# zkonduit/ezkl

Hardware: NVIDIA H100
Metric: prove_time_s (lower is better)
Workload: dtype u32 limbs (254-bit Montgomery integers mod BN254 r/p)

## Files before the change

ezkl_b200/csrc/field.cuh:

```cuda
#pragma once
#include <stdint.h>
#include "fp_ptx.cuh"

#if defined(__CUDACC__)
#define HD __host__ __device__ __forceinline__
#define DEV __device__ __forceinline__
#else
#define HD inline
#define DEV inline
#endif

namespace b200 {

struct FrTag {
    static constexpr uint32_t INV = 0xefffffffu;
    HD static uint32_t mod(int i) {
        constexpr uint32_t M[8] = {0xf0000001u, 0x43e1f593u, 0x79b97091u, 0x2833e848u, 0x8181585du, 0xb85045b6u, 0xe131a029u, 0x30644e72u};
        return M[i];
    }
    HD static uint32_t one(int i) {
        constexpr uint32_t V[8] = {0x4ffffffbu, 0xac96341cu, 0x9f60cd29u, 0x36fc7695u, 0x7879462eu, 0x666ea36fu, 0x9a07df2fu, 0x0e0a77c1u};
        return V[i];
    }
    HD static uint32_t r2(int i) {
// ... 180 lines not shown
    {
        uint64_t br = 2;
        for (int i = 0; i < 8; ++i) { uint64_t s = (uint64_t)Tag::mod(i) - br; e[i] = (uint32_t)s; br = (s >> 32) & 1; }
    }
    Fp<Tag> acc = fp_one<Tag>();
#pragma unroll 1
    for (int i = 253; i >= 0; --i) {
        acc = acc * acc;
        if ((e[i >> 5] >> (i & 31)) & 1) acc = acc * a;
    }
    return acc;
}
template <class Tag> HD Fp<Tag> fp_pow_u64(const Fp<Tag>& a, uint64_t e) {
    Fp<Tag> acc = fp_one<Tag>();
#pragma unroll 1
    for (int i = 63; i >= 0; --i) {
        acc = acc * acc;
        if ((e >> i) & 1) acc = acc * a;
    }
    return acc;
}

#if defined(__CUDACC__)
template <class Tag> DEV Fp<Tag> fp_load(const Fp<Tag>* p) {
    Fp<Tag> r;
    const uint4* q = reinterpret_cast<const uint4*>(p);
    uint4 lo = q[0], hi = q[1];
    r.l[0] = lo.x; r.l[1] = lo.y; r.l[2] = lo.z; r.l[3] = lo.w;
    r.l[4] = hi.x; r.l[5] = hi.y; r.l[6] = hi.z; r.l[7] = hi.w;
    return r;
}
template <class Tag> DEV void fp_store(Fp<Tag>* p, const Fp<Tag>& v) {
    uint4* q = reinterpret_cast<uint4*>(p);
    q[0] = make_uint4(v.l[0], v.l[1], v.l[2], v.l[3]);
    q[1] = make_uint4(v.l[4], v.l[5], v.l[6], v.l[7]);
}
#endif

}
```

ezkl_b200/csrc/fp_gen.py:

```python
#!/usr/bin/env python
import random
import sys

M32 = 0xFFFFFFFF
FIELDS = {
    "fr": 0x30644e72e131a029b85045b68181585d2833e84879b9709143e1f593f0000001,
    "fq": 0x30644e72e131a029b85045b68181585d97816a916871ca8d3c208c16d87cfd47,
}


def limbs(x, n=8):
    return [(x >> (32 * i)) & M32 for i in range(n)]


def gen_mul(mod):
    Ml = limbs(mod)
    inv = (-pow(mod, -1, 1 << 32)) & M32
    ins = []
    X = ["x%d" % i for i in range(8)]
    Y = ["y%d" % i for i in range(8)]
    A = ["a%d" % i for i in range(8)]
    B = ["b%d" % i for i in range(8)]

    def imm(v):
        return "0x%08x" % v

    def reduce_row(E, O):
        ins.append(("mul.lo.u32", "m", E[0], imm(inv)))
        for j in range(4):
            ins.append((("mad.lo.cc.u32" if j == 0 else "madc.lo.cc.u32"), O[2 * j], "m", imm(Ml[2 * j + 1]), O[2 * j]))
            ins.append(("madc.hi.cc.u32", O[2 * j + 1], "m", imm(Ml[2 * j + 1]), O[2 * j + 1]))
        for j in range(4):
            ins.append((("mad.lo.cc.u32" if j == 0 else "madc.lo.cc.u32"), E[2 * j], "m", imm(Ml[2 * j]), E[2 * j]))
            ins.append(("madc.hi.cc.u32", E[2 * j + 1], "m", imm(Ml[2 * j]), E[2 * j + 1]))
        ins.append(("addc.u32", O[7], O[7], "0"))

    for j in range(4):
        ins.append(("mul.lo.u32", X[2 * j], A[2 * j], B[0]))
        ins.append(("mul.hi.u32", X[2 * j + 1], A[2 * j], B[0]))
    for j in range(4):
        ins.append(("mul.lo.u32", Y[2 * j], A[2 * j + 1], B[0]))
        ins.append(("mul.hi.u32", Y[2 * j + 1], A[2 * j + 1], B[0]))
    E, O = X, Y
    reduce_row(E, O)
    for i in range(1, 8):
        nE, nO = O, E
        ins.append(("add.cc.u32", nE[0], nE[0], nO[1]))
        for j in range(4):
            c_lo = nO[2 * j + 2] if 2 * j + 2 < 8 else "0"
            c_hi = nO[2 * j + 3] if 2 * j + 3 < 8 else "0"
            ins.append(("madc.lo.cc.u32", nO[2 * j], A[2 * j + 1], B[i], c_lo))
            ins.append(("madc.hi.cc.u32", nO[2 * j + 1], A[2 * j + 1], B[i], c_hi))
        for j in range(4):
            ins.append((("mad.lo.cc.u32" if j == 0 else "madc.lo.cc.u32"), nE[2 * j], A[2 * j], B[i], nE[2 * j]))
            ins.append(("madc.hi.cc.u32", nE[2 * j + 1], A[2 * j], B[i], nE[2 * j + 1]))
        ins.append(("addc.u32", nO[7], nO[7], "0"))
        E, O = nE, nO
        reduce_row(E, O)
    T = ["t%d" % i for i in range(8)]
    for j in range(7):
        ins.append((("add.cc.u32" if j == 0 else "addc.cc.u32"), T[j], O[j], E[j + 1]))
    ins.append(("addc.u32", T[7], O[7], "0"))
    ins += final_sub(T, Ml)
    return ins


def gen_mul2(mod):
    Ml = limbs(mod)
    inv = (-pow(mod, -1, 1 << 32)) & M32
    ins = []
    X = ["x%d" % i for i in range(8)]
    Y = ["y%d" % i for i in range(8)]
    A = ["a%d" % i for i in range(8)]
    B = ["b%d" % i for i in range(8)]
    Cc = ["c%d" % i for i in range(8)]
    D = ["d%d" % i for i in range(8)]

    def imm(v):
        return "0x%08x" % v

    def acc_rows(E, O, P, q):
        def pair(p):
            return (q, p) if p.startswith("0x") else (p, q)
        for j in range(4):
            ins.append((("mad.lo.cc.u32" if j == 0 else "madc.lo.cc.u32"), O[2 * j]) + pair(P[2 * j + 1]) + (O[2 * j],))
            ins.append(("madc.hi.cc.u32", O[2 * j + 1]) + pair(P[2 * j + 1]) + (O[2 * j + 1],))
# ... 109 lines not shown


def final_sub(T, Ml, out=None):
    out = out or ["r%d" % i for i in range(8)]
    ins = []
    S = ["s%d" % i for i in range(8)]
    for j in range(8):
        ins.append((("sub.cc.u32" if j == 0 else "subc.cc.u32"), S[j], T[j], "0x%08x" % Ml[j]))
    ins.append(("subc.u32", "brw", "0", "0"))
    ins.append(("setp.eq.u32", "p", "brw", "0"))
    for j in range(8):
        ins.append(("selp.u32", out[j], S[j], T[j], "p"))
    return ins


def gen_add(mod):
    Ml = limbs(mod)
    ins = []
    T = ["t%d" % i for i in range(8)]
    for j in range(8):
        op = "add.cc.u32" if j == 0 else ("addc.cc.u32" if j < 7 else "addc.u32")
        ins.append((op, T[j], "a%d" % j, "b%d" % j))
    return ins + final_sub(T, Ml)


def gen_sub(mod):
    Ml = limbs(mod)
    ins = []
    T = ["t%d" % i for i in range(8)]
    for j in range(8):
        ins.append((("sub.cc.u32" if j == 0 else "subc.cc.u32"), T[j], "a%d" % j, "b%d" % j))
    ins.append(("subc.u32", "brw", "0", "0"))
    for j in range(8):
        ins.append(("and.b32", "s%d" % j, "brw", "0x%08x" % Ml[j]))
    for j in range(8):
        op = "add.cc.u32" if j == 0 else ("addc.cc.u32" if j < 7 else "addc.u32")
        ins.append((op, "r%d" % j, T[j], "s%d" % j))
    return ins


def run(ins, regs):
    cc = 0
    pred = {}

    def val(x):
        if x in regs:
# ... 4 lines not shown
        op, d = it[0], it[1]
        s = [val(x) if x not in pred else x for x in it[2:]]
        if op == "mul.lo.u32":
            regs[d] = (s[0] * s[1]) & M32
        elif op == "mul.hi.u32":
            regs[d] = (s[0] * s[1]) >> 32
        elif op in ("mad.lo.cc.u32", "madc.lo.cc.u32", "madc.hi.cc.u32", "mad.hi.cc.u32"):
            p = s[0] * s[1]
            p = (p & M32) if ".lo" in op else (p >> 32)
            t = p + s[2] + (cc if op.startswith("madc") else 0)
            regs[d], cc = t & M32, t >> 32
        elif op in ("add.cc.u32", "addc.cc.u32", "addc.u32"):
            t = s[0] + s[1] + (cc if op.startswith("addc") else 0)
            regs[d] = t & M32
            if ".cc" in op:
                cc = t >> 32
        elif op in ("sub.cc.u32", "subc.cc.u32", "subc.u32"):
            t = s[0] - s[1] - (cc if op.startswith("subc") else 0)
            regs[d] = t & M32
            if ".cc" in op:
                cc = 1 if t < 0 else 0
        elif op == "and.b32":
            regs[d] = s[0] & s[1]
        elif op == "shl.b32":
            regs[d] = (s[0] << s[1]) & M32
        elif op == "shf.l.clamp.b32":
            regs[d] = ((((s[1] << 32) | s[0]) << min(s[2], 32)) >> 32) & M32
        elif op == "setp.eq.u32":
            pred[d] = (s[0] == s[1])
        elif op == "selp.u32":
            regs[d] = s[0] if pred[it[4]] else s[1]
        else:
            raise ValueError(op)
        assert 0 <= regs.get(d, 0) <= M32
    return regs


def check(name, mod, trials=3000):
    rng = random.Random(hash(name) & 0xFFFF)
    mul, add, sub = gen_mul(mod), gen_add(mod), gen_sub(mod)
    Rinv = pow(1 << 256, -1, mod)
    edge = [0, 1, 2, mod - 1, mod - 2, (1 << 254) % mod, (1 << 253), mod >> 1, 0xFFFFFFFF, (1 << 128) - 1]
    pairs = [(x, y) for x in edge for y in edge] + [(rng.randrange(mod), rng.randrange(mod)) for _ in range(trials)]
    for a, b in pairs:
        regs = {}
        for i, v in enumerate(limbs(a)):
# ... 7 lines not shown
    mul2 = gen_mul2(mod)
    edge2 = [0, 1, mod - 1, mod, (1 << 254) % mod, 0xFFFFFFFF, mod >> 1]
    quads = [(a, b, c, d) for a in edge2 for b in edge2 for c in edge2 for d in edge2]
    quads += [tuple(rng.randrange(mod) for _ in range(4)) for _ in range(trials)]
    for a, b, c, d in quads:
        regs = {}
        for nm, v in (("a", a), ("b", b), ("c", c), ("d", d)):
            for i, w in enumerate(limbs(v)):
                regs["%s%d" % (nm, i)] = w
        out = run(mul2, regs)
        got = sum(out["r%d" % i] << (32 * i) for i in range(8))
        exp = (a * b + c * d) * Rinv % mod
        assert got == exp, (name, "mul2", hex(a), hex(b), hex(c), hex(d), hex(got), hex(exp))
    sqr = gen_sqr(mod)
    for a in edge + [mod, (1 << 254) - 1 if (1 << 254) - 1 < mod else mod - 3, 0x80000000, 0xFFFFFFFF << 32, int("80000000" * 8, 16) % mod,
                     int("ffffffff" * 7, 16)] + [rng.randrange(mod) for _ in range(trials)]:
        regs = {"a%d" % i: v for i, v in enumerate(limbs(a))}
        out = run(sqr, regs)
        got = sum(out["r%d" % i] << (32 * i) for i in range(8))
        assert got == a * a * Rinv % mod, (name, "sqr", hex(a), hex(got))
    return len(mul), len(add), len(sub), len(mul2), len(sqr)


def emit_fn(fname, ins, n_in):
    tmp = sorted({x for it in ins for x in it[1:] if x[0] in "xytsmuw" and not x.startswith("0x")} | {"brw"})
    tmp = [t for t in tmp if t != "p"]
    lines = ["    .reg .u32 %s;" % ", ".join(tmp), "    .reg .pred p;"]

    def opnd(x):
        if x[0] == "r" and x[1:].isdigit():
            return "%%%d" % int(x[1:])
        if x[0] == "a" and x[1:].isdigit():
            return "%%%d" % (8 + int(x[1:]))
        if x[0] == "b" and x[1:].isdigit() and x != "brw":
            return "%%%d" % (16 + int(x[1:]))
        if x[0] == "c" and x[1:].isdigit():
            return "%%%d" % (24 + int(x[1:]))
        if x[0] == "d" and x[1:].isdigit():
            return "%%%d" % (32 + int(x[1:]))
        return x

    for it in ins:
        lines.append("    %s %s;" % (it[0], ", ".join(opnd(x) for x in it[1:])))
    body = "\n".join('        "%s\\n\\t"' % ln.strip() for ln in ["{"] + lines + ["}"])
    outs = ", ".join('"=r"(r[%d])' % i for i in range(8))
    inps = ", ".join('"r"(a[%d])' % i for i in range(8))
    args = "uint32_t* r, const uint32_t* a"
    if n_in >= 2:
        inps += ", " + ", ".join('"r"(b[%d])' % i for i in range(8))
        args += ", const uint32_t* b"
    if n_in == 4:
        inps += ", " + ", ".join('"r"(c[%d])' % i for i in range(8)) + ", " + ", ".join('"r"(d[%d])' % i for i in range(8))
        args += ", const uint32_t* c, const uint32_t* d"
    return ("__device__ __forceinline__ void %s(%s) {\n    asm(\n%s\n        : %s\n        : %s);\n}\n"
            % (fname, args, body, outs, inps))


def main():
    out = ["// GENERATED by fp_gen.py -- do not edit.  Every instruction list below was executed by the generator's",
           "// PTX interpreter against Python bigints (edge + random operands) before this file was written.",
           "#pragma once", "#include <stdint.h>", "#if defined(__CUDA_ARCH__)", ""]
    for name, mod in FIELDS.items():
        n = check(name, mod)
        print("%s: verified; instruction counts mul/add/sub/mul2/sqr = %s" % (name, n))
        out.append(emit_fn("%s_mul_ptx" % name, gen_mul(mod), 2))
        out.append(emit_fn("%s_add_ptx" % name, gen_add(mod), 2))
        out.append(emit_fn("%s_sub_ptx" % name, gen_sub(mod), 2))
        out.append(emit_fn("%s_mul2_ptx" % name, gen_mul2(mod), 4))
        out.append(emit_fn("%s_sqr_ptx" % name, gen_sqr(mod), 1))
    out.append("#endif  // __CUDA_ARCH__")
    if "--check" not in sys.argv:
        import os
        with open(os.path.join(os.path.dirname(os.path.abspath(__file__)), "fp_ptx.cuh"), "w") as f:
            f.write("\n".join(out) + "\n")


if __name__ == "__main__":
    main()
```

ezkl_b200/csrc/fp_ptx.cuh:

```cuda
#pragma once
#include <stdint.h>
#if defined(__CUDA_ARCH__)

__device__ __forceinline__ void fr_mul_ptx(uint32_t* r, const uint32_t* a, const uint32_t* b) {
    asm(
        "{\n\t"
        ".reg .u32 brw, m, s0, s1, s2, s3, s4, s5, s6, s7, t0, t1, t2, t3, t4, t5, t6, t7, x0, x1, x2, x3, x4, x5, x6, x7, y0, y1, y2, y3, y4, y5, y6, y7;\n\t"
        ".reg .pred p;\n\t"
        "mul.lo.u32 x0, %8, %16;\n\t"
        "mul.hi.u32 x1, %8, %16;\n\t"
        "mul.lo.u32 x2, %10, %16;\n\t"
        "mul.hi.u32 x3, %10, %16;\n\t"
        "mul.lo.u32 x4, %12, %16;\n\t"
        "mul.hi.u32 x5, %12, %16;\n\t"
        "mul.lo.u32 x6, %14, %16;\n\t"
        "mul.hi.u32 x7, %14, %16;\n\t"
        "mul.lo.u32 y0, %9, %16;\n\t"
        "mul.hi.u32 y1, %9, %16;\n\t"
        "mul.lo.u32 y2, %11, %16;\n\t"
        "mul.hi.u32 y3, %11, %16;\n\t"
        "mul.lo.u32 y4, %13, %16;\n\t"
        "mul.hi.u32 y5, %13, %16;\n\t"
        "mul.lo.u32 y6, %15, %16;\n\t"
        "mul.hi.u32 y7, %15, %16;\n\t"
// ... 2262 lines not shown
        "sub.cc.u32 s0, t0, 0xd87cfd47;\n\t"
        "subc.cc.u32 s1, t1, 0x3c208c16;\n\t"
        "subc.cc.u32 s2, t2, 0x6871ca8d;\n\t"
        "subc.cc.u32 s3, t3, 0x97816a91;\n\t"
        "subc.cc.u32 s4, t4, 0x8181585d;\n\t"
        "subc.cc.u32 s5, t5, 0xb85045b6;\n\t"
        "subc.cc.u32 s6, t6, 0xe131a029;\n\t"
        "subc.cc.u32 s7, t7, 0x30644e72;\n\t"
        "subc.u32 brw, 0, 0;\n\t"
        "setp.eq.u32 p, brw, 0;\n\t"
        "selp.u32 %0, s0, t0, p;\n\t"
        "selp.u32 %1, s1, t1, p;\n\t"
        "selp.u32 %2, s2, t2, p;\n\t"
        "selp.u32 %3, s3, t3, p;\n\t"
        "selp.u32 %4, s4, t4, p;\n\t"
        "selp.u32 %5, s5, t5, p;\n\t"
        "selp.u32 %6, s6, t6, p;\n\t"
        "selp.u32 %7, s7, t7, p;\n\t"
        "}\n\t"
        : "=r"(r[0]), "=r"(r[1]), "=r"(r[2]), "=r"(r[3]), "=r"(r[4]), "=r"(r[5]), "=r"(r[6]), "=r"(r[7])
        : "r"(a[0]), "r"(a[1]), "r"(a[2]), "r"(a[3]), "r"(a[4]), "r"(a[5]), "r"(a[6]), "r"(a[7]));
}

#endif
```

ezkl_b200/csrc/ntt.cu:

```cuda
#include <cstdlib>
#include "ntt.cuh"

namespace b200 {

struct PassArgs {
    const Fr* src; Fr* dst;
    size_t src_pstride, dst_pstride;
    uint32_t logm, log_g, inner_cnt, in_r_fast;
    uint64_t in_rs, in_inner_s, in_outer_s;
    uint64_t out_rs, out_inner_s, out_outer_s;
    uint64_t n_in;
    uint32_t tw_on, rest_is_inner, lo_bits, first, last;
    uint64_t tw_mul;
    const Fr* tw_m; const Fr* t_lo; const Fr* t_hi;
    const uint4* tw_staged;
    const Fr* t_full;
    NttScale pre, post;
    uint32_t pre_c0_is_one;
    uint32_t peer_on, log_slice, block0;
    const Fr* src_peers[8];
    Fr* dst_peers[8];
};

DEV Fr sh_get(const uint4* lo, const uint4* hi, uint32_t i) {
// ... 117 lines not shown
    }

    int s = (int)a.logm - 1;
    bool first = true, tw_ready = false;
    while (s >= 0) {
        const bool two = !(first && (a.logm & 1u));
        const int s_next = two ? s - 2 : s - 1;
        const bool last = s_next < 0;
        uint32_t g, t;
        const bool g_fast = last || (first && !a.in_r_fast);
        if (g_fast) { g = tid & (G - 1); t = tid >> a.log_g; } else { t = tid & (Q - 1); g = tid >> (a.logm - 2); }
        const uint32_t q = 1u << (s - 1), p = t & (q - 1), blk = t >> (s - 1);
        const uint32_t base = (blk << (s + 1)) + p;
        Fr x[4];
        const bool sparse = first && a.first && a.n_in < ((uint64_t)M * a.inner_cnt);
        if (first) {
#pragma unroll
            for (int j = 0; j < 4; ++j) {
                const uint64_t idx = in_base + (uint64_t)g * a.in_inner_s + (uint64_t)(base + j * q) * a.in_rs;
                x[j] = fp_zero<FrTag>();
                if (idx < a.n_in) {
                    x[j] = fp_load(a.peer_on ? a.src_peers[idx >> a.log_slice] + (idx & slice_mask) : src + idx);
                    if (a.first) {
                        if (a.pre.mode == 1) x[j] = x[j] * a.pre.c[0];
                        else if (a.pre.mode == 3) { uint32_t m3 = (uint32_t)(idx % 3); if (m3 || !a.pre_c0_is_one) x[j] = x[j] * a.pre.c[m3]; }
                    }
                }
            }
        } else {
#pragma unroll
            for (int j = 0; j < 4; ++j) x[j] = sh_get(dlo, dhi, (g << a.logm) + base + j * q);
        }
        if (!tw_ready) { mbar_wait(&bar, 0); tw_ready = true; }
        {
            const uint32_t o = (1u << s) - 1u;
            Fr u0 = x[0] + x[2], u2 = x[0] - x[2], u1 = x[1] + x[3], u3 = x[1] - x[3];
            if (s > 0) {
                if (p && !(sparse && fp_is_zero(u2))) u2 = u2 * sh_get(tlo, thi, o + p);
                if (!(sparse && fp_is_zero(u3))) u3 = u3 * sh_get(tlo, thi, o + p + q);
            }
            x[0] = u0; x[1] = u1; x[2] = u2; x[3] = u3;
        }
        if (two) {
            const uint32_t o = (1u << (s - 1)) - 1u;
            Fr v0 = x[0] + x[1], v1 = x[0] - x[1], v2 = x[2] + x[3], v3 = x[2] - x[3];
            if (s - 1 > 0 && p) {
                Fr w = sh_get(tlo, thi, o + p);
                if (!(sparse && fp_is_zero(v1))) v1 = v1 * w;
                if (!(sparse && fp_is_zero(v3))) v3 = v3 * w;
            }
            x[0] = v0; x[1] = v1; x[2] = v2; x[3] = v3;
        }
        if (!last) {
#pragma unroll
            for (int j = 0; j < 4; ++j) sh_put(dlo, dhi, (g << a.logm) + base + j * q, x[j]);
            __syncthreads();
        } else {
#pragma unroll
            for (int j = 0; j < 4; ++j) {
                const uint32_t pos = base + j * q;
                const uint32_t rp = __brev(pos) >> (32 - a.logm);
                Fr v = x[j];
                if (a.tw_on) {
                    const uint64_t i_rest = a.rest_is_inner ? (uint64_t)(inner0 + g) : 0;
                    const uint64_t ex = a.tw_mul * (uint64_t)rp * i_rest;
                    if (ex) {
                        if (a.t_full) v = v * fp_load(a.t_full + ex);
                        else {
                            const uint32_t elo = (uint32_t)(ex & ((1ull << a.lo_bits) - 1)), ehi = (uint32_t)(ex >> a.lo_bits);
                            Fr w = fp_load(a.t_lo + elo);
                            if (ehi) w = w * fp_load(a.t_hi + ehi);
                            v = v * w;
                        }
                    }
                }
                const uint64_t idx = out_base + (uint64_t)g * a.out_inner_s + (uint64_t)rp * a.out_rs;
                if (a.last) {
                    if (a.post.mode == 1) v = v * a.post.c[0];
                    else if (a.post.mode == 3) v = v * a.post.c[(uint32_t)(idx % 3)];
                }
                fp_store(a.peer_on ? a.dst_peers[idx >> a.log_slice] + (idx & slice_mask) : dst + idx, v);
            }
        }
        first = false;
        s = s_next;
    }
}

__global__ void k_stage_twiddles(Fr w, uint32_t logm, uint4* __restrict__ out) {
    const uint32_t M = 1u << logm, idx = blockIdx.x * blockDim.x + threadIdx.x;
    if (idx >= M) return;
    Fr v = fp_zero<FrTag>();
    if (idx + 1 < M) {
        const uint32_t s = 31 - __clz(idx + 1), p = idx + 1 - (1u << s);
        v = fp_pow_u64(w, (uint64_t)p << (logm - 1 - s));
    }
    out[idx] = make_uint4(v.l[0], v.l[1], v.l[2], v.l[3]);
    out[M + idx] = make_uint4(v.l[4], v.l[5], v.l[6], v.l[7]);
}
__global__ void k_powers_run(Fr base, uint64_t count, Fr* __restrict__ out) {
    const uint64_t i0 = ((uint64_t)blockIdx.x * blockDim.x + threadIdx.x) * 32;
    if (i0 >= count) return;
    Fr v = fp_pow_u64(base, i0);
    for (uint64_t i = i0; i < i0 + 32 && i < count; ++i) { fp_store(out + i, v); v = v * base; }
// ... 177 lines not shown
```

Before: 0.08531.

## Use lazy [0,2r) Montgomery reduction in NTT butterflies, canonicalize on store

Adds generated PTX for lazy Fr arithmetic: Montgomery multiply without the final conditional subtraction, add and sub that keep results in [0,2r), a reduce-mod-2r and a canonicalize step. The NTT kernel's butterflies, twiddle multiplies and pre/post scaling now use these lazy ops, with one canonicalization before each global store. The aim is to drop the per-op compare-and-select against r and shorten the instruction count per butterfly. The cost is extra reduce2 calls on the untwiddled branches and reliance on redundant-range correctness, which the generator checks by simulation.

```diff
diff --git a/ezkl_b200/csrc/field.cuh b/ezkl_b200/csrc/field.cuh
--- a/ezkl_b200/csrc/field.cuh
+++ b/ezkl_b200/csrc/field.cuh
@@ -226,6 +226,42 @@
 }
 
 #if defined(__CUDACC__)
+DEV Fr fr_mul_lazy(const Fr& a, const Fr& b) {
+    Fr r;
+#if defined(__CUDA_ARCH__)
+    fr_mul_lazy_ptx(r.l, a.l, b.l);
+#endif
+    return r;
+}
+DEV Fr fr_add_lazy(const Fr& a, const Fr& b) {
+    Fr r;
+#if defined(__CUDA_ARCH__)
+    fr_add_lazy_ptx(r.l, a.l, b.l);
+#endif
+    return r;
+}
+DEV Fr fr_sub_lazy(const Fr& a, const Fr& b) {
+    Fr r;
+#if defined(__CUDA_ARCH__)
+    fr_sub_lazy_ptx(r.l, a.l, b.l);
+#endif
+    return r;
+}
+DEV Fr fr_reduce2(const Fr& a) {
+    Fr r;
+#if defined(__CUDA_ARCH__)
+    fr_reduce2_ptx(r.l, a.l);
+#endif
+    return r;
+}
+DEV Fr fr_canonicalize(const Fr& a) {
+    Fr r;
+#if defined(__CUDA_ARCH__)
+    fr_canonicalize_ptx(r.l, a.l);
+#endif
+    return r;
+}
+
 template <class Tag> DEV Fp<Tag> fp_load(const Fp<Tag>* p) {
     Fp<Tag> r;
     const uint4* q = reinterpret_cast<const uint4*>(p);
diff --git a/ezkl_b200/csrc/fp_gen.py b/ezkl_b200/csrc/fp_gen.py
--- a/ezkl_b200/csrc/fp_gen.py
+++ b/ezkl_b200/csrc/fp_gen.py
@@ -13,7 +13,7 @@
     return [(x >> (32 * i)) & M32 for i in range(n)]
 
 
-def gen_mul(mod):
+def gen_mul(mod, lazy=False):
     Ml = limbs(mod)
     inv = (-pow(mod, -1, 1 << 32)) & M32
     ins = []
@@ -57,11 +57,12 @@
         ins.append(("addc.u32", nO[7], nO[7], "0"))
         E, O = nE, nO
         reduce_row(E, O)
-    T = ["t%d" % i for i in range(8)]
+    T = ["r%d" % i for i in range(8)] if lazy else ["t%d" % i for i in range(8)]
     for j in range(7):
         ins.append((("add.cc.u32" if j == 0 else "addc.cc.u32"), T[j], O[j], E[j + 1]))
     ins.append(("addc.u32", T[7], O[7], "0"))
-    ins += final_sub(T, Ml)
+    if not lazy:
+        ins += final_sub(T, Ml)
     return ins
 
 
@@ -217,6 +218,33 @@
         op = "add.cc.u32" if j == 0 else ("addc.cc.u32" if j < 7 else "addc.u32")
         ins.append((op, T[j], "a%d" % j, "b%d" % j))
     return ins + final_sub(T, Ml)
+
+
+def gen_add_lazy(mod):
+    ins = []
+    T = ["t%d" % i for i in range(8)]
+    for j in range(8):
+        op = "add.cc.u32" if j == 0 else ("addc.cc.u32" if j < 7 else "addc.u32")
+        ins.append((op, T[j], "a%d" % j, "b%d" % j))
+    return ins + final_sub(T, limbs(2 * mod))
+
+
+def gen_sub_lazy(mod):
+    M2 = limbs(2 * mod)
+    ins = []
+    T = ["t%d" % i for i in range(8)]
+    for j in range(8):
+        op = "sub.cc.u32" if j == 0 else ("subc.cc.u32" if j < 7 else "subc.u32")
+        ins.append((op, T[j], "a%d" % j, "b%d" % j))
+    for j in range(8):
+        op = "add.cc.u32" if j == 0 else ("addc.cc.u32" if j < 7 else "addc.u32")
+        ins.append((op, "r%d" % j, T[j], "0x%08x" % M2[j]))
+    return ins
+
+
+def gen_reduce(mod, k):
+    T = ["t%d" % i for i in range(8)]
+    return [("mov.b32", T[j], "a%d" % j) for j in range(8)] + final_sub(T, limbs(k * mod))
 
 
 def gen_sub(mod):
@@ -267,6 +295,8 @@
                 cc = 1 if t < 0 else 0
         elif op == "and.b32":
             regs[d] = s[0] & s[1]
+        elif op == "mov.b32":
+            regs[d] = s[0]
         elif op == "shl.b32":
             regs[d] = (s[0] << s[1]) & M32
         elif op == "shf.l.clamp.b32":
@@ -320,6 +350,41 @@
     return len(mul), len(add), len(sub), len(mul2), len(sqr)
 
 
+def check_lazy(name, mod, trials=3000):
+    rng = random.Random((hash(name) + 1) & 0xFFFF)
+    Rinv = pow(1 << 256, -1, mod)
+    mul, add, sub = gen_mul(mod, lazy=True), gen_add_lazy(mod), gen_sub_lazy(mod)
+    red2, canon = gen_reduce(mod, 2), gen_reduce(mod, 1)
+    edge = [0, mod - 1, mod, 2 * mod - 1]
+    edge4 = edge + [2 * mod, 3 * mod, 4 * mod - 1]
+
+    def go(ins, **ops):
+        regs = {}
+        for nm, v in ops.items():
+            for i, w in enumerate(limbs(v)):
+                regs["%s%d" % (nm, i)] = w
+        out = run(ins, regs)
+        return sum(out["r%d" % i] << (32 * i) for i in range(8))
+
+    two = [(a, b) for a in edge for b in edge] + [(rng.randrange(2 * mod), rng.randrange(2 * mod)) for _ in range(trials)]
+    for a, b in two:
+        got = go(mul, a=a, b=b)
+        assert got < 2 * mod and got % mod == a * b * Rinv % mod, (name, "mul_lazy", hex(a), hex(b), hex(got))
+        got = go(add, a=a, b=b)
+        assert got < 2 * mod and got % mod == (a + b) % mod, (name, "add_lazy", hex(a), hex(b), hex(got))
+        got = go(sub, a=a, b=b)
+        assert got == a - b + 2 * mod, (name, "sub_lazy", hex(a), hex(b), hex(got))
+    wide = [(a, b) for a in edge4 for b in (0, 1, mod - 1)] + [(rng.randrange(4 * mod), rng.randrange(mod)) for _ in range(trials)]
+    for a, b in wide:
+        got = go(mul, a=a, b=b)
+        assert got < 2 * mod and got % mod == a * b * Rinv % mod, (name, "mul_lazy 4M", hex(a), hex(b), hex(got))
+    for a in edge4 + [rng.randrange(4 * mod) for _ in range(trials)]:
+        assert go(red2, a=a) == a % (2 * mod), (name, "reduce 2M", hex(a))
+        if a < 2 * mod:
+            assert go(canon, a=a) == a % mod, (name, "canonicalize", hex(a))
+    return len(mul), len(add), len(sub), len(red2), len(canon)
+
+
 def emit_fn(fname, ins, n_in):
     tmp = sorted({x for it in ins for x in it[1:] if x[0] in "xytsmuw" and not x.startswith("0x")} | {"brw"})
     tmp = [t for t in tmp if t != "p"]
@@ -366,6 +431,13 @@
         out.append(emit_fn("%s_sub_ptx" % name, gen_sub(mod), 2))
         out.append(emit_fn("%s_mul2_ptx" % name, gen_mul2(mod), 4))
         out.append(emit_fn("%s_sqr_ptx" % name, gen_sqr(mod), 1))
+    n = check_lazy("fr", FIELDS["fr"])
+    print("fr lazy: verified; instruction counts mul/add/sub/reduce2/canonicalize = %s" % (n,))
+    out.append(emit_fn("fr_mul_lazy_ptx", gen_mul(FIELDS["fr"], lazy=True), 2))
+    out.append(emit_fn("fr_add_lazy_ptx", gen_add_lazy(FIELDS["fr"]), 2))
+    out.append(emit_fn("fr_sub_lazy_ptx", gen_sub_lazy(FIELDS["fr"]), 2))
+    out.append(emit_fn("fr_reduce2_ptx", gen_reduce(FIELDS["fr"], 2), 1))
+    out.append(emit_fn("fr_canonicalize_ptx", gen_reduce(FIELDS["fr"], 1), 1))
     out.append("#endif  // __CUDA_ARCH__")
     if "--check" not in sys.argv:
         import os
diff --git a/ezkl_b200/csrc/fp_ptx.cuh b/ezkl_b200/csrc/fp_ptx.cuh
--- a/ezkl_b200/csrc/fp_ptx.cuh
+++ b/ezkl_b200/csrc/fp_ptx.cuh
@@ -2308,4 +2308,442 @@
         : "r"(a[0]), "r"(a[1]), "r"(a[2]), "r"(a[3]), "r"(a[4]), "r"(a[5]), "r"(a[6]), "r"(a[7]));
 }
 
+__device__ __forceinline__ void fr_mul_lazy_ptx(uint32_t* r, const uint32_t* a, const uint32_t* b) {
+    asm(
+        "{\n\t"
+        ".reg .u32 brw, m, x0, x1, x2, x3, x4, x5, x6, x7, y0, y1, y2, y3, y4, y5, y6, y7;\n\t"
+        ".reg .pred p;\n\t"
+        "mul.lo.u32 x0, %8, %16;\n\t"
+        "mul.hi.u32 x1, %8, %16;\n\t"
+        "mul.lo.u32 x2, %10, %16;\n\t"
+        "mul.hi.u32 x3, %10, %16;\n\t"
+        "mul.lo.u32 x4, %12, %16;\n\t"
+        "mul.hi.u32 x5, %12, %16;\n\t"
+        "mul.lo.u32 x6, %14, %16;\n\t"
+        "mul.hi.u32 x7, %14, %16;\n\t"
+        "mul.lo.u32 y0, %9, %16;\n\t"
+        "mul.hi.u32 y1, %9, %16;\n\t"
+        "mul.lo.u32 y2, %11, %16;\n\t"
+        "mul.hi.u32 y3, %11, %16;\n\t"
+        "mul.lo.u32 y4, %13, %16;\n\t"
+        "mul.hi.u32 y5, %13, %16;\n\t"
+        "mul.lo.u32 y6, %15, %16;\n\t"
+        "mul.hi.u32 y7, %15, %16;\n\t"
+        "mul.lo.u32 m, x0, 0xefffffff;\n\t"
+        "mad.lo.cc.u32 y0, m, 0x43e1f593, y0;\n\t"
+        "madc.hi.cc.u32 y1, m, 0x43e1f593, y1;\n\t"
+        "madc.lo.cc.u32 y2, m, 0x2833e848, y2;\n\t"
+        "madc.hi.cc.u32 y3, m, 0x2833e848, y3;\n\t"
+        "madc.lo.cc.u32 y4, m, 0xb85045b6, y4;\n\t"
+        "madc.hi.cc.u32 y5, m, 0xb85045b6, y5;\n\t"
+        "madc.lo.cc.u32 y6, m, 0x30644e72, y6;\n\t"
+        "madc.hi.cc.u32 y7, m, 0x30644e72, y7;\n\t"
+        "mad.lo.cc.u32 x0, m, 0xf0000001, x0;\n\t"
+        "madc.hi.cc.u32 x1, m, 0xf0000001, x1;\n\t"
+        "madc.lo.cc.u32 x2, m, 0x79b97091, x2;\n\t"
+        "madc.hi.cc.u32 x3, m, 0x79b97091, x3;\n\t"
+        "madc.lo.cc.u32 x4, m, 0x8181585d, x4;\n\t"
+        "madc.hi.cc.u32 x5, m, 0x8181585d, x5;\n\t"
+        "madc.lo.cc.u32 x6, m, 0xe131a029, x6;\n\t"
+        "madc.hi.cc.u32 x7, m, 0xe131a029, x7;\n\t"
+        "addc.u32 y7, y7, 0;\n\t"
+        "add.cc.u32 y0, y0, x1;\n\t"
+        "madc.lo.cc.u32 x0, %9, %17, x2;\n\t"
+        "madc.hi.cc.u32 x1, %9, %17, x3;\n\t"
+        "madc.lo.cc.u32 x2, %11, %17, x4;\n\t"
+        "madc.hi.cc.u32 x3, %11, %17, x5;\n\t"
+        "madc.lo.cc.u32 x4, %13, %17, x6;\n\t"
+        "madc.hi.cc.u32 x5, %13, %17, x7;\n\t"
+        "madc.lo.cc.u32 x6, %15, %17, 0;\n\t"
+        "madc.hi.cc.u32 x7, %15, %17, 0;\n\t"
+        "mad.lo.cc.u32 y0, %8, %17, y0;\n\t"
+        "madc.hi.cc.u32 y1, %8, %17, y1;\n\t"
+        "madc.lo.cc.u32 y2, %10, %17, y2;\n\t"
+        "madc.hi.cc.u32 y3, %10, %17, y3;\n\t"
+        "madc.lo.cc.u32 y4, %12, %17, y4;\n\t"
+        "madc.hi.cc.u32 y5, %12, %17, y5;\n\t"
+        "madc.lo.cc.u32 y6, %14, %17, y6;\n\t"
+        "madc.hi.cc.u32 y7, %14, %17, y7;\n\t"
+        "addc.u32 x7, x7, 0;\n\t"
+        "mul.lo.u32 m, y0, 0xefffffff;\n\t"
+        "mad.lo.cc.u32 x0, m, 0x43e1f593, x0;\n\t"
+        "madc.hi.cc.u32 x1, m, 0x43e1f593, x1;\n\t"
+        "madc.lo.cc.u32 x2, m, 0x2833e848, x2;\n\t"
+        "madc.hi.cc.u32 x3, m, 0x2833e848, x3;\n\t"
+        "madc.lo.cc.u32 x4, m, 0xb85045b6, x4;\n\t"
+        "madc.hi.cc.u32 x5, m, 0xb85045b6, x5;\n\t"
+        "madc.lo.cc.u32 x6, m, 0x30644e72, x6;\n\t"
+        "madc.hi.cc.u32 x7, m, 0x30644e72, x7;\n\t"
+        "mad.lo.cc.u32 y0, m, 0xf0000001, y0;\n\t"
+        "madc.hi.cc.u32 y1, m, 0xf0000001, y1;\n\t"
+        "madc.lo.cc.u32 y2, m, 0x79b97091, y2;\n\t"
+        "madc.hi.cc.u32 y3, m, 0x79b97091, y3;\n\t"
+        "madc.lo.cc.u32 y4, m, 0x8181585d, y4;\n\t"
+        "madc.hi.cc.u32 y5, m, 0x8181585d, y5;\n\t"
+        "madc.lo.cc.u32 y6, m, 0xe131a029, y6;\n\t"
+        "madc.hi.cc.u32 y7, m, 0xe131a029, y7;\n\t"
+        "addc.u32 x7, x7, 0;\n\t"
+        "add.cc.u32 x0, x0, y1;\n\t"
+        "madc.lo.cc.u32 y0, %9, %18, y2;\n\t"
+        "madc.hi.cc.u32 y1, %9, %18, y3;\n\t"
+        "madc.lo.cc.u32 y2, %11, %18, y4;\n\t"
+        "madc.hi.cc.u32 y3, %11, %18, y5;\n\t"
+        "madc.lo.cc.u32 y4, %13, %18, y6;\n\t"
+        "madc.hi.cc.u32 y5, %13, %18, y7;\n\t"
+        "madc.lo.cc.u32 y6, %15, %18, 0;\n\t"
+        "madc.hi.cc.u32 y7, %15, %18, 0;\n\t"
+        "mad.lo.cc.u32 x0, %8, %18, x0;\n\t"
+        "madc.hi.cc.u32 x1, %8, %18, x1;\n\t"
+        "madc.lo.cc.u32 x2, %10, %18, x2;\n\t"
+        "madc.hi.cc.u32 x3, %10, %18, x3;\n\t"
+        "madc.lo.cc.u32 x4, %12, %18, x4;\n\t"
+        "madc.hi.cc.u32 x5, %12, %18, x5;\n\t"
+        "madc.lo.cc.u32 x6, %14, %18, x6;\n\t"
+        "madc.hi.cc.u32 x7, %14, %18, x7;\n\t"
+        "addc.u32 y7, y7, 0;\n\t"
+        "mul.lo.u32 m, x0, 0xefffffff;\n\t"
+        "mad.lo.cc.u32 y0, m, 0x43e1f593, y0;\n\t"
+        "madc.hi.cc.u32 y1, m, 0x43e1f593, y1;\n\t"
+        "madc.lo.cc.u32 y2, m, 0x2833e848, y2;\n\t"
+        "madc.hi.cc.u32 y3, m, 0x2833e848, y3;\n\t"
+        "madc.lo.cc.u32 y4, m, 0xb85045b6, y4;\n\t"
+        "madc.hi.cc.u32 y5, m, 0xb85045b6, y5;\n\t"
+        "madc.lo.cc.u32 y6, m, 0x30644e72, y6;\n\t"
+        "madc.hi.cc.u32 y7, m, 0x30644e72, y7;\n\t"
+        "mad.lo.cc.u32 x0, m, 0xf0000001, x0;\n\t"
+        "madc.hi.cc.u32 x1, m, 0xf0000001, x1;\n\t"
+        "madc.lo.cc.u32 x2, m, 0x79b97091, x2;\n\t"
+        "madc.hi.cc.u32 x3, m, 0x79b97091, x3;\n\t"
+        "madc.lo.cc.u32 x4, m, 0x8181585d, x4;\n\t"
+        "madc.hi.cc.u32 x5, m, 0x8181585d, x5;\n\t"
+        "madc.lo.cc.u32 x6, m, 0xe131a029, x6;\n\t"
+        "madc.hi.cc.u32 x7, m, 0xe131a029, x7;\n\t"
+        "addc.u32 y7, y7, 0;\n\t"
+        "add.cc.u32 y0, y0, x1;\n\t"
+        "madc.lo.cc.u32 x0, %9, %19, x2;\n\t"
+        "madc.hi.cc.u32 x1, %9, %19, x3;\n\t"
+        "madc.lo.cc.u32 x2, %11, %19, x4;\n\t"
+        "madc.hi.cc.u32 x3, %11, %19, x5;\n\t"
+        "madc.lo.cc.u32 x4, %13, %19, x6;\n\t"
+        "madc.hi.cc.u32 x5, %13, %19, x7;\n\t"
+        "madc.lo.cc.u32 x6, %15, %19, 0;\n\t"
+        "madc.hi.cc.u32 x7, %15, %19, 0;\n\t"
+        "mad.lo.cc.u32 y0, %8, %19, y0;\n\t"
+        "madc.hi.cc.u32 y1, %8, %19, y1;\n\t"
+        "madc.lo.cc.u32 y2, %10, %19, y2;\n\t"
+        "madc.hi.cc.u32 y3, %10, %19, y3;\n\t"
+        "madc.lo.cc.u32 y4, %12, %19, y4;\n\t"
+        "madc.hi.cc.u32 y5, %12, %19, y5;\n\t"
+        "madc.lo.cc.u32 y6, %14, %19, y6;\n\t"
+        "madc.hi.cc.u32 y7, %14, %19, y7;\n\t"
+        "addc.u32 x7, x7, 0;\n\t"
+        "mul.lo.u32 m, y0, 0xefffffff;\n\t"
+        "mad.lo.cc.u32 x0, m, 0x43e1f593, x0;\n\t"
+        "madc.hi.cc.u32 x1, m, 0x43e1f593, x1;\n\t"
+        "madc.lo.cc.u32 x2, m, 0x2833e848, x2;\n\t"
+        "madc.hi.cc.u32 x3, m, 0x2833e848, x3;\n\t"
+        "madc.lo.cc.u32 x4, m, 0xb85045b6, x4;\n\t"
+        "madc.hi.cc.u32 x5, m, 0xb85045b6, x5;\n\t"
+        "madc.lo.cc.u32 x6, m, 0x30644e72, x6;\n\t"
+        "madc.hi.cc.u32 x7, m, 0x30644e72, x7;\n\t"
+        "mad.lo.cc.u32 y0, m, 0xf0000001, y0;\n\t"
+        "madc.hi.cc.u32 y1, m, 0xf0000001, y1;\n\t"
+        "madc.lo.cc.u32 y2, m, 0x79b97091, y2;\n\t"
+        "madc.hi.cc.u32 y3, m, 0x79b97091, y3;\n\t"
+        "madc.lo.cc.u32 y4, m, 0x8181585d, y4;\n\t"
+        "madc.hi.cc.u32 y5, m, 0x8181585d, y5;\n\t"
+        "madc.lo.cc.u32 y6, m, 0xe131a029, y6;\n\t"
+        "madc.hi.cc.u32 y7, m, 0xe131a029, y7;\n\t"
+        "addc.u32 x7, x7, 0;\n\t"
+        "add.cc.u32 x0, x0, y1;\n\t"
+        "madc.lo.cc.u32 y0, %9, %20, y2;\n\t"
+        "madc.hi.cc.u32 y1, %9, %20, y3;\n\t"
+        "madc.lo.cc.u32 y2, %11, %20, y4;\n\t"
+        "madc.hi.cc.u32 y3, %11, %20, y5;\n\t"
+        "madc.lo.cc.u32 y4, %13, %20, y6;\n\t"
+        "madc.hi.cc.u32 y5, %13, %20, y7;\n\t"
+        "madc.lo.cc.u32 y6, %15, %20, 0;\n\t"
+        "madc.hi.cc.u32 y7, %15, %20, 0;\n\t"
+        "mad.lo.cc.u32 x0, %8, %20, x0;\n\t"
+        "madc.hi.cc.u32 x1, %8, %20, x1;\n\t"
+        "madc.lo.cc.u32 x2, %10, %20, x2;\n\t"
+        "madc.hi.cc.u32 x3, %10, %20, x3;\n\t"
+        "madc.lo.cc.u32 x4, %12, %20, x4;\n\t"
+        "madc.hi.cc.u32 x5, %12, %20, x5;\n\t"
+        "madc.lo.cc.u32 x6, %14, %20, x6;\n\t"
+        "madc.hi.cc.u32 x7, %14, %20, x7;\n\t"
+        "addc.u32 y7, y7, 0;\n\t"
+        "mul.lo.u32 m, x0, 0xefffffff;\n\t"
+        "mad.lo.cc.u32 y0, m, 0x43e1f593, y0;\n\t"
+        "madc.hi.cc.u32 y1, m, 0x43e1f593, y1;\n\t"
+        "madc.lo.cc.u32 y2, m, 0x2833e848, y2;\n\t"
+        "madc.hi.cc.u32 y3, m, 0x2833e848, y3;\n\t"
+        "madc.lo.cc.u32 y4, m, 0xb85045b6, y4;\n\t"
+        "madc.hi.cc.u32 y5, m, 0xb85045b6, y5;\n\t"
+        "madc.lo.cc.u32 y6, m, 0x30644e72, y6;\n\t"
+        "madc.hi.cc.u32 y7, m, 0x30644e72, y7;\n\t"
+        "mad.lo.cc.u32 x0, m, 0xf0000001, x0;\n\t"
+        "madc.hi.cc.u32 x1, m, 0xf0000001, x1;\n\t"
+        "madc.lo.cc.u32 x2, m, 0x79b97091, x2;\n\t"
+        "madc.hi.cc.u32 x3, m, 0x79b97091, x3;\n\t"
+        "madc.lo.cc.u32 x4, m, 0x8181585d, x4;\n\t"
+        "madc.hi.cc.u32 x5, m, 0x8181585d, x5;\n\t"
+        "madc.lo.cc.u32 x6, m, 0xe131a029, x6;\n\t"
+        "madc.hi.cc.u32 x7, m, 0xe131a029, x7;\n\t"
+        "addc.u32 y7, y7, 0;\n\t"
+        "add.cc.u32 y0, y0, x1;\n\t"
+        "madc.lo.cc.u32 x0, %9, %21, x2;\n\t"
+        "madc.hi.cc.u32 x1, %9, %21, x3;\n\t"
+        "madc.lo.cc.u32 x2, %11, %21, x4;\n\t"
+        "madc.hi.cc.u32 x3, %11, %21, x5;\n\t"
+        "madc.lo.cc.u32 x4, %13, %21, x6;\n\t"
+        "madc.hi.cc.u32 x5, %13, %21, x7;\n\t"
+        "madc.lo.cc.u32 x6, %15, %21, 0;\n\t"
+        "madc.hi.cc.u32 x7, %15, %21, 0;\n\t"
+        "mad.lo.cc.u32 y0, %8, %21, y0;\n\t"
+        "madc.hi.cc.u32 y1, %8, %21, y1;\n\t"
+        "madc.lo.cc.u32 y2, %10, %21, y2;\n\t"
+        "madc.hi.cc.u32 y3, %10, %21, y3;\n\t"
+        "madc.lo.cc.u32 y4, %12, %21, y4;\n\t"
+        "madc.hi.cc.u32 y5, %12, %21, y5;\n\t"
+        "madc.lo.cc.u32 y6, %14, %21, y6;\n\t"
+        "madc.hi.cc.u32 y7, %14, %21, y7;\n\t"
+        "addc.u32 x7, x7, 0;\n\t"
+        "mul.lo.u32 m, y0, 0xefffffff;\n\t"
+        "mad.lo.cc.u32 x0, m, 0x43e1f593, x0;\n\t"
+        "madc.hi.cc.u32 x1, m, 0x43e1f593, x1;\n\t"
+        "madc.lo.cc.u32 x2, m, 0x2833e848, x2;\n\t"
+        "madc.hi.cc.u32 x3, m, 0x2833e848, x3;\n\t"
+        "madc.lo.cc.u32 x4, m, 0xb85045b6, x4;\n\t"
+        "madc.hi.cc.u32 x5, m, 0xb85045b6, x5;\n\t"
+        "madc.lo.cc.u32 x6, m, 0x30644e72, x6;\n\t"
+        "madc.hi.cc.u32 x7, m, 0x30644e72, x7;\n\t"
+        "mad.lo.cc.u32 y0, m, 0xf0000001, y0;\n\t"
+        "madc.hi.cc.u32 y1, m, 0xf0000001, y1;\n\t"
+        "madc.lo.cc.u32 y2, m, 0x79b97091, y2;\n\t"
+        "madc.hi.cc.u32 y3, m, 0x79b97091, y3;\n\t"
+        "madc.lo.cc.u32 y4, m, 0x8181585d, y4;\n\t"
+        "madc.hi.cc.u32 y5, m, 0x8181585d, y5;\n\t"
+        "madc.lo.cc.u32 y6, m, 0xe131a029, y6;\n\t"
+        "madc.hi.cc.u32 y7, m, 0xe131a029, y7;\n\t"
+        "addc.u32 x7, x7, 0;\n\t"
+        "add.cc.u32 x0, x0, y1;\n\t"
+        "madc.lo.cc.u32 y0, %9, %22, y2;\n\t"
+        "madc.hi.cc.u32 y1, %9, %22, y3;\n\t"
+        "madc.lo.cc.u32 y2, %11, %22, y4;\n\t"
+        "madc.hi.cc.u32 y3, %11, %22, y5;\n\t"
+        "madc.lo.cc.u32 y4, %13, %22, y6;\n\t"
+        "madc.hi.cc.u32 y5, %13, %22, y7;\n\t"
+        "madc.lo.cc.u32 y6, %15, %22, 0;\n\t"
+        "madc.hi.cc.u32 y7, %15, %22, 0;\n\t"
+        "mad.lo.cc.u32 x0, %8, %22, x0;\n\t"
+        "madc.hi.cc.u32 x1, %8, %22, x1;\n\t"
+        "madc.lo.cc.u32 x2, %10, %22, x2;\n\t"
+        "madc.hi.cc.u32 x3, %10, %22, x3;\n\t"
+        "madc.lo.cc.u32 x4, %12, %22, x4;\n\t"
+        "madc.hi.cc.u32 x5, %12, %22, x5;\n\t"
+        "madc.lo.cc.u32 x6, %14, %22, x6;\n\t"
+        "madc.hi.cc.u32 x7, %14, %22, x7;\n\t"
+        "addc.u32 y7, y7, 0;\n\t"
+        "mul.lo.u32 m, x0, 0xefffffff;\n\t"
+        "mad.lo.cc.u32 y0, m, 0x43e1f593, y0;\n\t"
+        "madc.hi.cc.u32 y1, m, 0x43e1f593, y1;\n\t"
+        "madc.lo.cc.u32 y2, m, 0x2833e848, y2;\n\t"
+        "madc.hi.cc.u32 y3, m, 0x2833e848, y3;\n\t"
+        "madc.lo.cc.u32 y4, m, 0xb85045b6, y4;\n\t"
+        "madc.hi.cc.u32 y5, m, 0xb85045b6, y5;\n\t"
+        "madc.lo.cc.u32 y6, m, 0x30644e72, y6;\n\t"
+        "madc.hi.cc.u32 y7, m, 0x30644e72, y7;\n\t"
+        "mad.lo.cc.u32 x0, m, 0xf0000001, x0;\n\t"
+        "madc.hi.cc.u32 x1, m, 0xf0000001, x1;\n\t"
+        "madc.lo.cc.u32 x2, m, 0x79b97091, x2;\n\t"
+        "madc.hi.cc.u32 x3, m, 0x79b97091, x3;\n\t"
+        "madc.lo.cc.u32 x4, m, 0x8181585d, x4;\n\t"
+        "madc.hi.cc.u32 x5, m, 0x8181585d, x5;\n\t"
+        "madc.lo.cc.u32 x6, m, 0xe131a029, x6;\n\t"
+        "madc.hi.cc.u32 x7, m, 0xe131a029, x7;\n\t"
+        "addc.u32 y7, y7, 0;\n\t"
+        "add.cc.u32 y0, y0, x1;\n\t"
+        "madc.lo.cc.u32 x0, %9, %23, x2;\n\t"
+        "madc.hi.cc.u32 x1, %9, %23, x3;\n\t"
+        "madc.lo.cc.u32 x2, %11, %23, x4;\n\t"
+        "madc.hi.cc.u32 x3, %11, %23, x5;\n\t"
+        "madc.lo.cc.u32 x4, %13, %23, x6;\n\t"
+        "madc.hi.cc.u32 x5, %13, %23, x7;\n\t"
+        "madc.lo.cc.u32 x6, %15, %23, 0;\n\t"
+        "madc.hi.cc.u32 x7, %15, %23, 0;\n\t"
+        "mad.lo.cc.u32 y0, %8, %23, y0;\n\t"
+        "madc.hi.cc.u32 y1, %8, %23, y1;\n\t"
+        "madc.lo.cc.u32 y2, %10, %23, y2;\n\t"
+        "madc.hi.cc.u32 y3, %10, %23, y3;\n\t"
+        "madc.lo.cc.u32 y4, %12, %23, y4;\n\t"
+        "madc.hi.cc.u32 y5, %12, %23, y5;\n\t"
+        "madc.lo.cc.u32 y6, %14, %23, y6;\n\t"
+        "madc.hi.cc.u32 y7, %14, %23, y7;\n\t"
+        "addc.u32 x7, x7, 0;\n\t"
+        "mul.lo.u32 m, y0, 0xefffffff;\n\t"
+        "mad.lo.cc.u32 x0, m, 0x43e1f593, x0;\n\t"
+        "madc.hi.cc.u32 x1, m, 0x43e1f593, x1;\n\t"
+        "madc.lo.cc.u32 x2, m, 0x2833e848, x2;\n\t"
+        "madc.hi.cc.u32 x3, m, 0x2833e848, x3;\n\t"
+        "madc.lo.cc.u32 x4, m, 0xb85045b6, x4;\n\t"
+        "madc.hi.cc.u32 x5, m, 0xb85045b6, x5;\n\t"
+        "madc.lo.cc.u32 x6, m, 0x30644e72, x6;\n\t"
+        "madc.hi.cc.u32 x7, m, 0x30644e72, x7;\n\t"
+        "mad.lo.cc.u32 y0, m, 0xf0000001, y0;\n\t"
+        "madc.hi.cc.u32 y1, m, 0xf0000001, y1;\n\t"
+        "madc.lo.cc.u32 y2, m, 0x79b97091, y2;\n\t"
+        "madc.hi.cc.u32 y3, m, 0x79b97091, y3;\n\t"
+        "madc.lo.cc.u32 y4, m, 0x8181585d, y4;\n\t"
+        "madc.hi.cc.u32 y5, m, 0x8181585d, y5;\n\t"
+        "madc.lo.cc.u32 y6, m, 0xe131a029, y6;\n\t"
+        "madc.hi.cc.u32 y7, m, 0xe131a029, y7;\n\t"
+        "addc.u32 x7, x7, 0;\n\t"
+        "add.cc.u32 %0, x0, y1;\n\t"
+        "addc.cc.u32 %1, x1, y2;\n\t"
+        "addc.cc.u32 %2, x2, y3;\n\t"
+        "addc.cc.u32 %3, x3, y4;\n\t"
+        "addc.cc.u32 %4, x4, y5;\n\t"
+        "addc.cc.u32 %5, x5, y6;\n\t"
+        "addc.cc.u32 %6, x6, y7;\n\t"
+        "addc.u32 %7, x7, 0;\n\t"
+        "}\n\t"
+        : "=r"(r[0]), "=r"(r[1]), "=r"(r[2]), "=r"(r[3]), "=r"(r[4]), "=r"(r[5]), "=r"(r[6]), "=r"(r[7])
+        : "r"(a[0]), "r"(a[1]), "r"(a[2]), "r"(a[3]), "r"(a[4]), "r"(a[5]), "r"(a[6]), "r"(a[7]), "r"(b[0]), "r"(b[1]), "r"(b[2]), "r"(b[3]), "r"(b[4]), "r"(b[5]), "r"(b[6]), "r"(b[7]));
+}
+
+__device__ __forceinline__ void fr_add_lazy_ptx(uint32_t* r, const uint32_t* a, const uint32_t* b) {
+    asm(
+        "{\n\t"
+        ".reg .u32 brw, s0, s1, s2, s3, s4, s5, s6, s7, t0, t1, t2, t3, t4, t5, t6, t7;\n\t"
+        ".reg .pred p;\n\t"
+        "add.cc.u32 t0, %8, %16;\n\t"
+        "addc.cc.u32 t1, %9, %17;\n\t"
+        "addc.cc.u32 t2, %10, %18;\n\t"
+        "addc.cc.u32 t3, %11, %19;\n\t"
+        "addc.cc.u32 t4, %12, %20;\n\t"
+        "addc.cc.u32 t5, %13, %21;\n\t"
+        "addc.cc.u32 t6, %14, %22;\n\t"
+        "addc.u32 t7, %15, %23;\n\t"
+        "sub.cc.u32 s0, t0, 0xe0000002;\n\t"
+        "subc.cc.u32 s1, t1, 0x87c3eb27;\n\t"
+        "subc.cc.u32 s2, t2, 0xf372e122;\n\t"
+        "subc.cc.u32 s3, t3, 0x5067d090;\n\t"
+        "subc.cc.u32 s4, t4, 0x0302b0ba;\n\t"
+        "subc.cc.u32 s5, t5, 0x70a08b6d;\n\t"
+        "subc.cc.u32 s6, t6, 0xc2634053;\n\t"
+        "subc.cc.u32 s7, t7, 0x60c89ce5;\n\t"
+        "subc.u32 brw, 0, 0;\n\t"
+        "setp.eq.u32 p, brw, 0;\n\t"
+        "selp.u32 %0, s0, t0, p;\n\t"
+        "selp.u32 %1, s1, t1, p;\n\t"
+        "selp.u32 %2, s2, t2, p;\n\t"
+        "selp.u32 %3, s3, t3, p;\n\t"
+        "selp.u32 %4, s4, t4, p;\n\t"
+        "selp.u32 %5, s5, t5, p;\n\t"
+        "selp.u32 %6, s6, t6, p;\n\t"
+        "selp.u32 %7, s7, t7, p;\n\t"
+        "}\n\t"
+        : "=r"(r[0]), "=r"(r[1]), "=r"(r[2]), "=r"(r[3]), "=r"(r[4]), "=r"(r[5]), "=r"(r[6]), "=r"(r[7])
+        : "r"(a[0]), "r"(a[1]), "r"(a[2]), "r"(a[3]), "r"(a[4]), "r"(a[5]), "r"(a[6]), "r"(a[7]), "r"(b[0]), "r"(b[1]), "r"(b[2]), "r"(b[3]), "r"(b[4]), "r"(b[5]), "r"(b[6]), "r"(b[7]));
+}
+
+__device__ __forceinline__ void fr_sub_lazy_ptx(uint32_t* r, const uint32_t* a, const uint32_t* b) {
+    asm(
+        "{\n\t"
+        ".reg .u32 brw, t0, t1, t2, t3, t4, t5, t6, t7;\n\t"
+        ".reg .pred p;\n\t"
+        "sub.cc.u32 t0, %8, %16;\n\t"
+        "subc.cc.u32 t1, %9, %17;\n\t"
+        "subc.cc.u32 t2, %10, %18;\n\t"
+        "subc.cc.u32 t3, %11, %19;\n\t"
+        "subc.cc.u32 t4, %12, %20;\n\t"
+        "subc.cc.u32 t5, %13, %21;\n\t"
+        "subc.cc.u32 t6, %14, %22;\n\t"
+        "subc.u32 t7, %15, %23;\n\t"
+        "add.cc.u32 %0, t0, 0xe0000002;\n\t"
+        "addc.cc.u32 %1, t1, 0x87c3eb27;\n\t"
+        "addc.cc.u32 %2, t2, 0xf372e122;\n\t"
+        "addc.cc.u32 %3, t3, 0x5067d090;\n\t"
+        "addc.cc.u32 %4, t4, 0x0302b0ba;\n\t"
+        "addc.cc.u32 %5, t5, 0x70a08b6d;\n\t"
+        "addc.cc.u32 %6, t6, 0xc2634053;\n\t"
+        "addc.u32 %7, t7, 0x60c89ce5;\n\t"
+        "}\n\t"
+        : "=r"(r[0]), "=r"(r[1]), "=r"(r[2]), "=r"(r[3]), "=r"(r[4]), "=r"(r[5]), "=r"(r[6]), "=r"(r[7])
+        : "r"(a[0]), "r"(a[1]), "r"(a[2]), "r"(a[3]), "r"(a[4]), "r"(a[5]), "r"(a[6]), "r"(a[7]), "r"(b[0]), "r"(b[1]), "r"(b[2]), "r"(b[3]), "r"(b[4]), "r"(b[5]), "r"(b[6]), "r"(b[7]));
+}
+
+__device__ __forceinline__ void fr_reduce2_ptx(uint32_t* r, const uint32_t* a) {
+    asm(
+        "{\n\t"
+        ".reg .u32 brw, s0, s1, s2, s3, s4, s5, s6, s7, t0, t1, t2, t3, t4, t5, t6, t7;\n\t"
+        ".reg .pred p;\n\t"
+        "mov.b32 t0, %8;\n\t"
+        "mov.b32 t1, %9;\n\t"
+        "mov.b32 t2, %10;\n\t"
+        "mov.b32 t3, %11;\n\t"
+        "mov.b32 t4, %12;\n\t"
+        "mov.b32 t5, %13;\n\t"
+        "mov.b32 t6, %14;\n\t"
+        "mov.b32 t7, %15;\n\t"
+        "sub.cc.u32 s0, t0, 0xe0000002;\n\t"
+        "subc.cc.u32 s1, t1, 0x87c3eb27;\n\t"
+        "subc.cc.u32 s2, t2, 0xf372e122;\n\t"
+        "subc.cc.u32 s3, t3, 0x5067d090;\n\t"
+        "subc.cc.u32 s4, t4, 0x0302b0ba;\n\t"
+        "subc.cc.u32 s5, t5, 0x70a08b6d;\n\t"
+        "subc.cc.u32 s6, t6, 0xc2634053;\n\t"
+        "subc.cc.u32 s7, t7, 0x60c89ce5;\n\t"
+        "subc.u32 brw, 0, 0;\n\t"
+        "setp.eq.u32 p, brw, 0;\n\t"
+        "selp.u32 %0, s0, t0, p;\n\t"
+        "selp.u32 %1, s1, t1, p;\n\t"
+        "selp.u32 %2, s2, t2, p;\n\t"
+        "selp.u32 %3, s3, t3, p;\n\t"
+        "selp.u32 %4, s4, t4, p;\n\t"
+        "selp.u32 %5, s5, t5, p;\n\t"
+        "selp.u32 %6, s6, t6, p;\n\t"
+        "selp.u32 %7, s7, t7, p;\n\t"
+        "}\n\t"
+        : "=r"(r[0]), "=r"(r[1]), "=r"(r[2]), "=r"(r[3]), "=r"(r[4]), "=r"(r[5]), "=r"(r[6]), "=r"(r[7])
+        : "r"(a[0]), "r"(a[1]), "r"(a[2]), "r"(a[3]), "r"(a[4]), "r"(a[5]), "r"(a[6]), "r"(a[7]));
+}
+
+__device__ __forceinline__ void fr_canonicalize_ptx(uint32_t* r, const uint32_t* a) {
+    asm(
+        "{\n\t"
+        ".reg .u32 brw, s0, s1, s2, s3, s4, s5, s6, s7, t0, t1, t2, t3, t4, t5, t6, t7;\n\t"
+        ".reg .pred p;\n\t"
+        "mov.b32 t0, %8;\n\t"
+        "mov.b32 t1, %9;\n\t"
+        "mov.b32 t2, %10;\n\t"
+        "mov.b32 t3, %11;\n\t"
+        "mov.b32 t4, %12;\n\t"
+        "mov.b32 t5, %13;\n\t"
+        "mov.b32 t6, %14;\n\t"
+        "mov.b32 t7, %15;\n\t"
+        "sub.cc.u32 s0, t0, 0xf0000001;\n\t"
+        "subc.cc.u32 s1, t1, 0x43e1f593;\n\t"
+        "subc.cc.u32 s2, t2, 0x79b97091;\n\t"
+        "subc.cc.u32 s3, t3, 0x2833e848;\n\t"
+        "subc.cc.u32 s4, t4, 0x8181585d;\n\t"
+        "subc.cc.u32 s5, t5, 0xb85045b6;\n\t"
+        "subc.cc.u32 s6, t6, 0xe131a029;\n\t"
+        "subc.cc.u32 s7, t7, 0x30644e72;\n\t"
+        "subc.u32 brw, 0, 0;\n\t"
+        "setp.eq.u32 p, brw, 0;\n\t"
+        "selp.u32 %0, s0, t0, p;\n\t"
+        "selp.u32 %1, s1, t1, p;\n\t"
+        "selp.u32 %2, s2, t2, p;\n\t"
+        "selp.u32 %3, s3, t3, p;\n\t"
+        "selp.u32 %4, s4, t4, p;\n\t"
+        "selp.u32 %5, s5, t5, p;\n\t"
+        "selp.u32 %6, s6, t6, p;\n\t"
+        "selp.u32 %7, s7, t7, p;\n\t"
+        "}\n\t"
+        : "=r"(r[0]), "=r"(r[1]), "=r"(r[2]), "=r"(r[3]), "=r"(r[4]), "=r"(r[5]), "=r"(r[6]), "=r"(r[7])
+        : "r"(a[0]), "r"(a[1]), "r"(a[2]), "r"(a[3]), "r"(a[4]), "r"(a[5]), "r"(a[6]), "r"(a[7]));
+}
+
 #endif
diff --git a/ezkl_b200/csrc/ntt.cu b/ezkl_b200/csrc/ntt.cu
--- a/ezkl_b200/csrc/ntt.cu
+++ b/ezkl_b200/csrc/ntt.cu
@@ -163,8 +163,8 @@
                 if (idx < a.n_in) {
                     x[j] = fp_load(a.peer_on ? a.src_peers[idx >> a.log_slice] + (idx & slice_mask) : src + idx);
                     if (a.first) {
-                        if (a.pre.mode == 1) x[j] = x[j] * a.pre.c[0];
-                        else if (a.pre.mode == 3) { uint32_t m3 = (uint32_t)(idx % 3); if (m3 || !a.pre_c0_is_one) x[j] = x[j] * a.pre.c[m3]; }
+                        if (a.pre.mode == 1) x[j] = fr_mul_lazy(x[j], a.pre.c[0]);
+                        else if (a.pre.mode == 3) { uint32_t m3 = (uint32_t)(idx % 3); if (m3 || !a.pre_c0_is_one) x[j] = fr_mul_lazy(x[j], a.pre.c[m3]); }
                     }
                 }
             }
@@ -175,20 +175,24 @@
         if (!tw_ready) { mbar_wait(&bar, 0); tw_ready = true; }
         {
             const uint32_t o = (1u << s) - 1u;
-            Fr u0 = x[0] + x[2], u2 = x[0] - x[2], u1 = x[1] + x[3], u3 = x[1] - x[3];
-            if (s > 0) {
-                if (p && !(sparse && fp_is_zero(u2))) u2 = u2 * sh_get(tlo, thi, o + p);
-                if (!(sparse && fp_is_zero(u3))) u3 = u3 * sh_get(tlo, thi, o + p + q);
-            }
+            Fr u0 = fr_add_lazy(x[0], x[2]), u2 = fr_sub_lazy(x[0], x[2]), u1 = fr_add_lazy(x[1], x[3]), u3 = fr_sub_lazy(x[1], x[3]);
+            if (s > 0 && p && !(sparse && fp_eq(x[0], x[2]))) u2 = fr_mul_lazy(u2, sh_get(tlo, thi, o + p));
+            else u2 = fr_reduce2(u2);
+            if (s > 0 && !(sparse && fp_eq(x[1], x[3]))) u3 = fr_mul_lazy(u3, sh_get(tlo, thi, o + p + q));
+            else u3 = fr_reduce2(u3);
             x[0] = u0; x[1] = u1; x[2] = u2; x[3] = u3;
         }
         if (two) {
             const uint32_t o = (1u << (s - 1)) - 1u;
-            Fr v0 = x[0] + x[1], v1 = x[0] - x[1], v2 = x[2] + x[3], v3 = x[2] - x[3];
+            Fr v0 = fr_add_lazy(x[0], x[1]), v1 = fr_sub_lazy(x[0], x[1]), v2 = fr_add_lazy(x[2], x[3]), v3 = fr_sub_lazy(x[2], x[3]);
             if (s - 1 > 0 && p) {
                 Fr w = sh_get(tlo, thi, o + p);
-                if (!(sparse && fp_is_zero(v1))) v1 = v1 * w;
-                if (!(sparse && fp_is_zero(v3))) v3 = v3 * w;
+                if (!(sparse && fp_eq(x[0], x[1]))) v1 = fr_mul_lazy(v1, w);
+                else v1 = fr_reduce2(v1);
+                if (!(sparse && fp_eq(x[2], x[3]))) v3 = fr_mul_lazy(v3, w);
+                else v3 = fr_reduce2(v3);
+            } else {
+                v1 = fr_reduce2(v1); v3 = fr_reduce2(v3);
             }
             x[0] = v0; x[1] = v1; x[2] = v2; x[3] = v3;
         }
@@ -206,21 +210,21 @@
                     const uint64_t i_rest = a.rest_is_inner ? (uint64_t)(inner0 + g) : 0;
                     const uint64_t ex = a.tw_mul * (uint64_t)rp * i_rest;
                     if (ex) {
-                        if (a.t_full) v = v * fp_load(a.t_full + ex);
+                        if (a.t_full) v = fr_mul_lazy(v, fp_load(a.t_full + ex));
                         else {
                             const uint32_t elo = (uint32_t)(ex & ((1ull << a.lo_bits) - 1)), ehi = (uint32_t)(ex >> a.lo_bits);
                             Fr w = fp_load(a.t_lo + elo);
-                            if (ehi) w = w * fp_load(a.t_hi + ehi);
-                            v = v * w;
+                            if (ehi) w = fr_mul_lazy(w, fp_load(a.t_hi + ehi));
+                            v = fr_mul_lazy(v, w);
                         }
                     }
                 }
                 const uint64_t idx = out_base + (uint64_t)g * a.out_inner_s + (uint64_t)rp * a.out_rs;
                 if (a.last) {
-                    if (a.post.mode == 1) v = v * a.post.c[0];
-                    else if (a.post.mode == 3) v = v * a.post.c[(uint32_t)(idx % 3)];
+                    if (a.post.mode == 1) v = fr_mul_lazy(v, a.post.c[0]);
+                    else if (a.post.mode == 3) v = fr_mul_lazy(v, a.post.c[(uint32_t)(idx % 3)]);
                 }
-                fp_store(a.peer_on ? a.dst_peers[idx >> a.log_slice] + (idx & slice_mask) : dst + idx, v);
+                fp_store(a.peer_on ? a.dst_peers[idx >> a.log_slice] + (idx & slice_mask) : dst + idx, fr_canonicalize(v));
             }
         }
         first = false;
```

Measured after the change: 0.08525, median of 6. No clear change (-0.1%).
